# KhutornoyYaroslav/vcm-ts

Measured on AMD Instinct MI355X. Metric: encoded frames/sec at 1920x1080 GOP-32, higher is better.
Workload: dtype f32 (fp16x3 split-MFMA, fp32 accumulate)

## Files before the change

### include/dcvc_hip.h

```cpp
#ifndef DCVC_HIP_H
#define DCVC_HIP_H

#include <stdint.h>

#ifdef __cplusplus
extern "C" {
#endif

#define DCVC_OK 0
#define DCVC_E_ARG (-1)
#define DCVC_E_LAUNCH (-2)
#define DCVC_E_RANGE (-3)

#define DCVC_STATUS_ACT_SATURATED 1

#define DCVC_MAX_SEG 3

#define DCVC_PREC_FP32 0
#define DCVC_PREC_FP16X3 1

typedef struct {
    const float *ptr;
    int32_t C;
    int32_t cs;
} dcvc_seg;

typedef struct {
    dcvc_seg seg[DCVC_MAX_SEG];
    int32_t nseg;
    int32_t N, Hin, Win;
    int32_t in_act;
    float in_slope;
    const float *wpack;
    const float *bpack;
    int32_t ks;
    int32_t stride;
    int32_t Cout;
    int32_t Cout_pad;
    float *out;
    int32_t out_cs;
    int32_t out_act;
    float out_slope;
    int32_t pixel_shuffle;
    const float *res;
    int32_t res_cs;
    const float *res_gate;
    const float *res2;
    int32_t res2_cs;
    int32_t precision;
    int32_t *status;
    float *chan_partial;
    int32_t tile_row0;
    int32_t tile_rows;
    int32_t pair_taps;
} dcvc_conv_args;

int32_t dcvc_conv_tile_rows(int32_t ks, int32_t stride);

int32_t dcvc_conv_chan_partial_parts(int32_t ks, int32_t stride, int32_t Hout, int32_t Wout);
int dcvc_channel_mean_finish(const float *chan_partial, int32_t parts, int32_t row_stride, float *mean, int32_t N,
                             int32_t C, int32_t HW, void *stream);

int64_t dcvc_conv_pack_size(int32_t Cout, int32_t ks, int32_t nseg, const int32_t *seg_C, int32_t *cout_pad);

int dcvc_conv_pack_weights(const float *w, const float *b, int32_t Cout, int32_t ks, int32_t nseg,
                           const int32_t *seg_C, int32_t pixel_shuffle, int32_t precision, float *wpack,
                           float *bpack);

int64_t dcvc_conv_pack_size_paired(int32_t Cout, int32_t Cin, int32_t *cout_pad);
int dcvc_conv_pack_weights_paired(const float *w, const float *b, int32_t Cout, int32_t Cin, float *wpack, float *bpack);

int dcvc_conv2d(const dcvc_conv_args *a, void *stream);
int dcvc_conv_set_lookahead(int32_t mode);

int64_t dcvc_conv_small_pack_bytes(int32_t Cout, int32_t ks, int32_t nseg, const int32_t *seg_C);
int dcvc_conv_small_pack_weights(const float *w, const float *b, int32_t Cout, int32_t ks, int32_t nseg,
                                 const int32_t *seg_C, void *wpack, float *bpack);
int dcvc_conv2d_small(const dcvc_conv_args *a, void *stream);

int64_t dcvc_conv_k32_pack_bytes(int32_t Cout, int32_t ks, int32_t nseg, const int32_t *seg_C, int32_t *cout_pad);
int dcvc_conv_k32_pack_weights(const float *w, const float *b, int32_t Cout, int32_t ks, int32_t nseg,
                               const int32_t *seg_C, int32_t pixel_shuffle, void *wpack, float *bpack);
int dcvc_conv2d_k32(const dcvc_conv_args *a, void *stream);
int dcvc_conv_k32_set_waves(int32_t waves);

int dcvc_warp(const float *src, int32_t src_cs, const float *flow, int32_t flow_cs, float *out, int32_t out_cs,
              int32_t N, int32_t H, int32_t W, int32_t C, void *stream);
int dcvc_up2(const float *src, int32_t src_cs, float *out, int32_t out_cs, float *out2, int32_t out2_cs,
             int32_t N, int32_t H, int32_t W, int32_t C, float scale, void *stream);
int dcvc_down2(const float *src, int32_t src_cs, float *out, int32_t out_cs, int32_t N, int32_t H, int32_t W,
               int32_t C, float scale, int32_t avgpool_order, void *stream);
int dcvc_maxpool2(const float *src, int32_t src_cs, float *out, int32_t out_cs, int32_t N, int32_t H, int32_t W,
                  int32_t C, void *stream);
int dcvc_copy_channels(const float *src, int32_t src_cs, float *out, int32_t out_cs, int64_t npix, int32_t C,
                       void *stream);
int dcvc_nchw_to_nhwc(const float *src, float *out, int32_t out_cs, int32_t N, int32_t C, int32_t H, int32_t W,
                      void *stream);
int dcvc_nhwc_to_nchw(const float *src, int32_t src_cs, float *out, int32_t N, int32_t C, int32_t H, int32_t W,
                      int32_t clamp01, void *stream);

int dcvc_channel_mean(const float *src, int32_t src_cs, float *mean, float *scratch, int32_t N, int32_t HW,
                      int32_t C, void *stream);
int dcvc_se_gate(const float *mean, const float *w1, const float *w2, float *gate, int32_t N, int32_t C,
                 int32_t Cr, void *stream);

int dcvc_scale_channels(const float *src, int32_t src_cs, float *out, int32_t out_cs, const float *q_basic,
                        const float *q_scale, int32_t mode, int32_t N, int32_t HW, int32_t C, void *stream);
int dcvc_scale_channels_map(const float *src, int32_t src_cs, float *out, int32_t out_cs, const float *q_basic,
                            const float *q_scale, int32_t mode, int32_t N, int32_t HW, int32_t C, const float *q_map,
                            int32_t H, int32_t W, void *stream);
int dcvc_round_symbols(const float *z, int32_t z_cs, float *z_hat, int32_t zh_cs, int32_t *sym, int32_t N,
                       int32_t H, int32_t W, int32_t C, void *stream);
int dcvc_symbols_to_nhwc(const int32_t *sym, float *out, int32_t out_cs, int32_t N, int32_t H, int32_t W,
                         int32_t C, void *stream);

typedef struct {
    const float *y;
    int32_t y_cs;
    const float *fusion;
    int32_t fusion_cs;
    const float *spatial;
    int32_t spatial_cs;
    float *params;
    int32_t params_cs;
    float *y_hat;
    float *y_q;
    float *y_res;
    float *scales_hat;
    int32_t *sym;
    int32_t *idx;
    float *out;
    int32_t out_cs;
    const float *q_basic;
    const float *q_scale;
    int32_t N, H, W, C;
    int32_t step;
    const float *idx_edges;
    const float *forced_q;
    const float *q_map;
} dcvc_dual_prior_args;

int dcvc_scale_indexes(const float *scales, int32_t *idx, int64_t n, const float *idx_edges, void *stream);

int dcvc_dual_prior_enc(const dcvc_dual_prior_args *a, void *stream);
int dcvc_dual_prior_dec_index(const dcvc_dual_prior_args *a, void *stream);
int dcvc_dual_prior_dec_apply(const dcvc_dual_prior_args *a, void *stream);

int dcvc_scale_bits(const float *y_q, const float *scales_hat, float *out, float *scratch, int32_t kind, int32_t N,
                    int64_t per_sample, void *stream);
int dcvc_factorized_bits(const float *z_hat, int32_t z_cs, const float *params, float *out, float *scratch, int32_t N,
                         int32_t HW, int32_t C, void *stream);
int dcvc_sq_err(const float *a, int32_t a_cs, const float *b, int32_t b_cs, float *out, float *scratch, int32_t N,
                int32_t HW, int32_t C, void *stream);

int32_t dcvc_cdf_table_cols(void);
int dcvc_build_scale_cdfs(const float *scales, int32_t n_scales, int32_t kind, int32_t *cdf, int32_t *sizes,
// ... 10 lines not shown
```

### vcm_ts_amd/csrc/conv_mfma.hip

```cpp
#include <hip/hip_runtime.h>
#include <stdint.h>
#include <stdlib.h>
#include <string.h>
#include <type_traits>
#include <vector>

#include "dcvc_hip.h"
#include "kernel_common.h"

namespace {

constexpr int LDK = 20;


struct ConvK {
    const float *seg_ptr[DCVC_MAX_SEG];
    int seg_C[DCVC_MAX_SEG];
    int seg_cs[DCVC_MAX_SEG];
    int nseg;
    int Hin, Win, Hout, Wout;
    int in_act;
    float in_slope;
    const float *wpack;
    const float *bpack;
    int Cout, Cout_pad;
    float *out;
    int out_cs;
    int out_act;
    float out_slope;
    int ps;
    const float *res;
    int res_cs;
    const float *res_gate;
    const float *res2;
    int res2_cs;
    int vec_epi;
    int *status;
    float *chan_partial;
    int ntx;
    int ty0, nty;
    int band_rows;
};

int g_lookahead = 2;

inline long dev_env_long(const char *name, long dflt) {
    const char *dev = getenv("DCVC_DEV");
    if (!dev || strcmp(dev, "1") != 0) return dflt;
    const char *v = getenv(name);
    return v ? atol(v) : dflt;
}


template <int KS, int S, int RPW, int NT, bool SPLIT, bool PAIR = false, bool AHEAD = false>
__global__ __launch_bounds__(256, 2) void conv_mfma(const ConvK a) {
    static_assert(!PAIR || (KS == 7 && S == 1 && SPLIT), "tap pairing is built for the 7x7 split-fp16 layers");
    constexpr int BH = 4 * RPW, BW = 32, BN = 32 * NT;
    constexpr int PH = (BH - 1) * S + KS, PW = (BW - 1) * S + KS, PAD = KS / 2;
    constexpr int T = PAIR ? KS * 4 : KS * KS;
    constexpr int TPS = PAIR ? 4 : (KS == 3 && S == 1) ? 9 : KS;
    constexpr int NST = T / TPS;
    constexpr int EPI_LD = BN + 4;
    constexpr int LDS_MAIN = PH * PW * LDK + TPS * 4 * BN * 4, LDS_EPI = 4 * 32 * EPI_LD, LDS_RED = 4 * BN;
    __shared__ __attribute__((aligned(16))) float lds[LDS_MAIN > LDS_EPI + LDS_RED ? LDS_MAIN : LDS_EPI + LDS_RED];
    float *patch = lds;
    float *wl = lds + PH * PW * LDK;

    const int tid = threadIdx.x, lane = tid & 63, wave = tid >> 6;
    const int nbn = a.Cout_pad / BN;
    const int nb = blockIdx.x % nbn, tx = blockIdx.x / nbn;
    if (tx >= a.ntx) return;
    const int ty = blockIdx.y + a.ty0;
    const int x0 = tx * BW, y0 = ty * BH, n0 = nb * BN, img = blockIdx.z;

    f32x16 acc[RPW][NT];
#pragma unroll
    for (int m = 0; m < RPW; ++m)
#pragma unroll
        for (int n = 0; n < NT; ++n)
#pragma unroll
            for (int r = 0; r < 16; ++r) acc[m][n][r] = 0.f;

    const int a_base = ((wave * RPW * S) * PW + (lane & 31) * S) * LDK + (lane >> 5) * 4;
    const int b_base = ((lane >> 5) * BN + (lane & 31)) * 4;

    constexpr int NP = (PH * PW * 4 + 255) / 256, NW = (TPS * 4 * BN + 255) / 256;
    static_assert(!AHEAD || NST >= 3, "AHEAD: two straight-line steps and a loop over the rest of a chunk");
    f32x4 rp[NP], rw[NW];
    struct Cursor {
        int s, c0, cg, st;
    };
    auto advance = [&](Cursor &k) {
        if (++k.st == NST) {
            k.st = 0;
            ++k.cg;
            k.c0 += MFMA_KC;
            if (k.c0 >= a.seg_C[k.s]) {
                ++k.s;
                k.c0 = 0;
            }
        }
    };
    int poff[NP];
    unsigned inpic = 0;
#pragma unroll
    for (int u = 0; u < NP; ++u) {
        const int i = tid + u * 256;
        const int p = i >> 2;
        const int py = p / PW, px = p - py * PW + (PAIR ? (i & 3) >> 1 : 0);
        const int gy = y0 * S - PAD + py, gx = x0 * S - PAD + px;
        const bool ok = i < PH * PW * 4 && gy >= 0 && gy < a.Hin && gx >= 0 && gx < a.Win;
        poff[u] = ok ? gy * a.Win + gx : 0;
        inpic |= (ok ? 1u : 0u) << u;
    }
    auto load_patch = [&](const Cursor &k) {
        const int C = a.seg_C[k.s], cs = a.seg_cs[k.s];
        const float *sp = a.seg_ptr[k.s] + (size_t)img * a.Hin * a.Win * cs;
        const int c = PAIR ? (tid & 1) * 4 : k.c0 + (tid & 3) * 4;
        const int cc = c < C ? c : 0;
#pragma unroll
        for (int u = 0; u < NP; ++u) rp[u] = *(const f32x4 *)(sp + (size_t)poff[u] * cs + cc);
    };
    auto store_patch = [&](const Cursor &k) {
        const int C = a.seg_C[k.s];
#pragma unroll
        for (int u = 0; u < NP; ++u) {
            const int i = tid + u * 256;
            if (i < PH * PW * 4) {
                const int c = PAIR ? (i & 1) * 4 : k.c0 + (i & 3) * 4;
                f32x4 v = ((inpic >> u) & 1u) && c < C ? rp[u] : (f32x4){0.f, 0.f, 0.f, 0.f};
                if (c + 3 >= C) {
                    if (c + 1 >= C) v[1] = 0.f;
                    if (c + 2 >= C) v[2] = 0.f;
                    v[3] = 0.f;
                }
                if (a.in_act) {
                    v[0] = act(v[0], a.in_slope);
                    v[1] = act(v[1], a.in_slope);
                    v[2] = act(v[2], a.in_slope);
                    v[3] = act(v[3], a.in_slope);
                }
                if (!SPLIT) {
                    *(f32x4 *)&patch[(i >> 2) * LDK + (i & 3) * 4] = v;
                } else {
                    f32x4 sv = v * ACT_SCALE;
#pragma unroll
                    for (int e = 0; e < 4; ++e) sv[e] = __builtin_amdgcn_fmed3f(sv[e], -F16_MAX, F16_MAX);
                    const f16x4 hi = __builtin_convertvector(sv, f16x4);
                    const f16x4 lo = __builtin_convertvector(sv - __builtin_convertvector(hi, f32x4), f16x4);
                    _Float16 *rec = (_Float16 *)&patch[(i >> 2) * LDK];
                    *(f16x4 *)&rec[(i & 3) * 4] = hi;
                    *(f16x4 *)&rec[16 + (i & 3) * 4] = lo;
                }
            }
        }
    };
    constexpr int W_OVER = NW * 256 - TPS * 4 * BN;
    static_assert(!AHEAD || TPS * 4 * BN >= W_OVER, "the doubled float4 must lie inside the slab");
    auto w_slot = [&](const int u) {
        const int i = tid + u * 256;
        return AHEAD && W_OVER > 0 && u == NW - 1 && i >= TPS * 4 * BN ? i - W_OVER : i;
    };
    auto load_w = [&](const Cursor &k) {
        const float *wsrc = a.wpack + ((size_t)(k.cg * T + k.st * TPS) * 4) * a.Cout_pad * 4 + (size_t)n0 * 4;
#pragma unroll
        for (int u = 0; u < NW; ++u) {
            const int i = w_slot(u);
            const int row = i / BN, col = i - row * BN;
            if (AHEAD || i < TPS * 4 * BN) rw[u] = *(const f32x4 *)(wsrc + ((size_t)row * a.Cout_pad + col) * 4);
        }
    };
    auto store_w = [&]() {
#pragma unroll
        for (int u = 0; u < NW; ++u) {
            const int i = w_slot(u);
            if (AHEAD || i < TPS * 4 * BN) *(f32x4 *)&wl[i * 4] = rw[u];
        }
    };
    auto mfma_step = [&](const int st) {
        const int a_st = (TPS == T) ? 0 : st * PW * LDK;
#pragma unroll
        for (int tt = 0; tt < TPS; ++tt) {
            const int ky = (TPS == T) ? tt / KS : 0, kx = PAIR ? 2 * tt : (TPS == T) ? tt % KS : tt;
            if (!SPLIT) {
#pragma unroll
                for (int k2 = 0; k2 < 2; ++k2) {
                    f32x4 af[RPW], bf[NT];
#pragma unroll
                    for (int m = 0; m < RPW; ++m)
                        af[m] = *(const f32x4 *)&patch[a_base + a_st + ((m * S + ky) * PW + kx) * LDK + k2 * 8];
#pragma unroll
                    for (int n = 0; n < NT; ++n)
                        bf[n] = *(const f32x4 *)&wl[b_base + ((tt * 4 + k2 * 2) * BN + n * 32) * 4];
#pragma unroll
                    for (int j = 0; j < 4; ++j)
#pragma unroll
                        for (int m = 0; m < RPW; ++m)
#pragma unroll
                            for (int n = 0; n < NT; ++n)
                                acc[m][n] = __builtin_amdgcn_mfma_f32_32x32x2f32(af[m][j], bf[n][j], acc[m][n], 0, 0, 0);
                }
            } else {
                f16x8 ah[RPW], al[RPW], bh[NT], bl[NT];
#pragma unroll
                for (int m = 0; m < RPW; ++m) {
                    const float *rec = &patch[a_base + a_st + ((m * S + ky) * PW + kx) * LDK];
                    ah[m] = *(const f16x8 *)rec;
                    al[m] = *(const f16x8 *)(rec + 8);
                }
#pragma unroll
                for (int n = 0; n < NT; ++n) {
                    bh[n] = *(const f16x8 *)&wl[b_base + ((tt * 4) * BN + n * 32) * 4];
                    bl[n] = *(const f16x8 *)&wl[b_base + ((tt * 4 + 2) * BN + n * 32) * 4];
                }
#pragma unroll
                for (int m = 0; m < RPW; ++m)
#pragma unroll
                    for (int n = 0; n < NT; ++n) {
                        acc[m][n] = __builtin_amdgcn_mfma_f32_32x32x16_f16(ah[m], bh[n], acc[m][n], 0, 0, 0);
                        acc[m][n] = __builtin_amdgcn_mfma_f32_32x32x16_f16(ah[m], bl[n], acc[m][n], 0, 0, 0);
                        acc[m][n] = __builtin_amdgcn_mfma_f32_32x32x16_f16(al[m], bh[n], acc[m][n], 0, 0, 0);
                    }
            }
        }
    };

    Cursor cur = {0, 0, 0, 0};
    if constexpr (AHEAD) {
        auto chunk = [&](auto more, const Cursor &nc) {
            constexpr bool MORE = decltype(more)::value;
            __syncthreads();
            store_patch(cur);
            store_w();
            __syncthreads();
            advance(cur);
            load_w(cur);
            if (MORE) load_patch(nc);
            mfma_step(0);
            auto row_step = [&](const int st) {
                __syncthreads();
                store_w();
                __syncthreads();
                if (st + 1 < NST) {
                    advance(cur);
                    load_w(cur);
                } else if (MORE) {
                    load_w(nc);
                }
                mfma_step(st);
            };
            row_step(1);
            for (int st = 2; st < NST; ++st) row_step(st);
        };
        load_patch(cur);
        load_w(cur);
        for (;;) {
            Cursor nc = cur;
            nc.st = NST - 1;
            advance(nc);
            if (nc.s >= a.nseg) break;
            chunk(std::true_type{}, nc);
            cur = nc;
        }
        chunk(std::false_type{}, cur);
    } else {
        load_patch(cur);
        load_w(cur);
        while (cur.s < a.nseg) {
            __syncthreads();
            if (cur.st == 0) store_patch(cur);
            store_w();
            __syncthreads();
            Cursor nxt = cur;
            advance(nxt);
            if (nxt.s < a.nseg) {
                if (nxt.st == 0) load_patch(nxt);
                load_w(nxt);
            }
            mfma_step(cur.st);
            cur = nxt;
        }
    }

    const int col = lane & 31, hh = lane >> 5;
    const int Cq = a.Cout >> 2;
    const int Cfin = a.ps ? Cq : a.Cout;
    const int Ho = a.ps ? a.Hout * 2 : a.Hout, Wo = a.ps ? a.Wout * 2 : a.Wout;
    const float inv_scale = SPLIT ? 1.f / (ACT_SCALE * WGT_SCALE) : 1.f;
    float vmax = 0.f;
    if (a.vec_epi) {
        constexpr int LPP = BN / 4, PPI = 64 / LPP, NIT = 32 / PPI;
        float *epi = lds + wave * 32 * EPI_LD;
        const int c4 = (lane % LPP) * 4, pl = lane / LPP;
        const int ch = n0 + c4;
        const bool ch_ok = ch < a.Cout;
        int dy = 0, dx = 0, cf = ch;
        if (a.ps) {
            const int sub = ch / Cq;
            cf = ch - sub * Cq;
            dy = sub >> 1;
            dx = sub & 1;
        }
        f32x4 bias = {0.f, 0.f, 0.f, 0.f}, gate = {1.f, 1.f, 1.f, 1.f};
        if (ch_ok) {
            bias = *(const f32x4 *)&a.bpack[ch];
            if (a.res_gate) gate = *(const f32x4 *)&a.res_gate[(size_t)img * Cfin + cf];
        }
        __syncthreads();
        size_t pix[RPW][NIT];
        bool ok[RPW][NIT];
        f32x4 rv[RPW][NIT], rv2[RPW][NIT];
// ... 57 lines not shown
            }
            asm volatile("s_waitcnt lgkmcnt(0)" ::: "memory");
        }
        if (a.status && !(vmax <= ACT_LIMIT)) atomicOr(a.status, DCVC_STATUS_ACT_SATURATED);
        if (a.chan_partial) {
#pragma unroll
            for (int off = LPP; off < 64; off <<= 1)
#pragma unroll
                for (int e = 0; e < 4; ++e) csum[e] += __shfl_xor(csum[e], off);
            float *red = lds + LDS_EPI;
            if (lane < LPP) *(f32x4 *)&red[wave * BN + c4] = csum;
            __syncthreads();
            if (tid < BN && n0 + tid < a.Cout_pad) {
                const float s = ((red[tid] + red[BN + tid]) + red[2 * BN + tid]) + red[3 * BN + tid];
                const size_t part = (size_t)img * (a.nty * a.ntx) + (size_t)ty * a.ntx + tx;
                a.chan_partial[part * a.Cout_pad + n0 + tid] = s;
            }
        }
        return;
    }
#pragma unroll
    for (int m = 0; m < RPW; ++m) {
        const int oy = y0 + wave * RPW + m;
        if (oy >= a.Hout) continue;
#pragma unroll
        for (int n = 0; n < NT; ++n) {
            const int ch = n0 + n * 32 + col;
            if (ch >= a.Cout) continue;
            const float bias = a.bpack[ch];
            int dy = 0, dx = 0, cf = ch;
            if (a.ps) {
                const int sub = ch / Cq;
                cf = ch - sub * Cq;
                dy = sub >> 1;
                dx = sub & 1;
            }
            const float gate = a.res_gate ? a.res_gate[(size_t)img * Cfin + cf] : 1.f;
            float rv[16], rv2[16];
#pragma unroll
            for (int r = 0; r < 16; ++r) {
                const int ox = x0 + (r & 3) + 8 * (r >> 2) + 4 * hh;
                const size_t pix = a.ps ? ((size_t)(img * Ho + 2 * oy + dy) * Wo + 2 * ox + dx)
                                        : ((size_t)(img * Ho + oy) * Wo + ox);
                rv[r] = (a.res && ox < a.Wout) ? a.res[pix * a.res_cs + cf] : 0.f;
                rv2[r] = (a.res2 && ox < a.Wout) ? a.res2[pix * a.res2_cs + cf] : 0.f;
            }
#pragma unroll
            for (int r = 0; r < 16; ++r) {
                const int ox = x0 + (r & 3) + 8 * (r >> 2) + 4 * hh;
                if (ox >= a.Wout) continue;
                float v = acc[m][n][r] * inv_scale + bias;
                if (a.out_act == 1) v = act(v, a.out_slope);
                else if (a.out_act == 2) v = fminf(fmaxf(v, 0.f), 1.f);
                const size_t pix = a.ps ? ((size_t)(img * Ho + 2 * oy + dy) * Wo + 2 * ox + dx)
                                        : ((size_t)(img * Ho + oy) * Wo + ox);
                if (a.out_act == 3) {
                    const float mk = rv2[r] > 0.f ? 1.f : a.out_slope;
                    v = a.res ? __builtin_fmaf(v, mk, rv[r]) : v * mk;
                } else {
                    if (a.res) v = a.res_gate ? __builtin_fmaf(rv[r], gate, v) : v + rv[r];
                    if (a.res2) v = rv2[r] + v;
                }
                if (a.status) vmax = fmaxf(vmax, fabsf(v));
                a.out[pix * a.out_cs + cf] = v;
            }
        }
    }
    if (a.status && !(vmax <= ACT_LIMIT)) atomicOr(a.status, DCVC_STATUS_ACT_SATURATED);
}


template <int KS, int S, int RPW, int NT, bool PAIR = false>
int launch(ConvK &k, int N, hipStream_t st, int precision) {
    constexpr int BH = 4 * RPW, BN = 32 * NT;
    k.ntx = (k.Wout + 31) / 32;
    static const bool xcd_pad = dev_env_long("DCVC_XCD_PAD", 0) != 0;
    unsigned gx = (unsigned)(k.ntx * (k.Cout_pad / BN));
    if (xcd_pad && gx >= 8) gx = (gx + 7) & ~7u;
    k.nty = (k.Hout + BH - 1) / BH;
    if (k.ty0 < 0 || k.ty0 >= k.nty) return DCVC_E_ARG;
    const int rows = k.band_rows > 0 ? (k.band_rows < k.nty - k.ty0 ? k.band_rows : k.nty - k.ty0) : k.nty;
    dim3 grid(gx, (unsigned)rows, (unsigned)N);
    constexpr bool HAS_AHEAD = (KS == 3 && S == 2) || KS == 7;
    if constexpr (HAS_AHEAD) {
        if (g_lookahead == 2) {
            if (PAIR)
                hipLaunchKernelGGL((conv_mfma<KS, S, RPW, NT, true, PAIR, true>), grid, dim3(256), 0, st, k);
            else if (precision == DCVC_PREC_FP16X3)
                hipLaunchKernelGGL((conv_mfma<KS, S, RPW, NT, true, false, true>), grid, dim3(256), 0, st, k);
            else
                hipLaunchKernelGGL((conv_mfma<KS, S, RPW, NT, false, false, !(KS == 7 && RPW == 2 && NT == 2)>), grid, dim3(256), 0, st, k);
            RET_LAUNCH();
        }
    }
    if (PAIR)
        hipLaunchKernelGGL((conv_mfma<KS, S, RPW, NT, true, PAIR>), grid, dim3(256), 0, st, k);
    else if (precision == DCVC_PREC_FP16X3)
        hipLaunchKernelGGL((conv_mfma<KS, S, RPW, NT, true>), grid, dim3(256), 0, st, k);
    else
        hipLaunchKernelGGL((conv_mfma<KS, S, RPW, NT, false>), grid, dim3(256), 0, st, k);
    RET_LAUNCH();
}

}

extern "C" int64_t dcvc_conv_pack_size(int32_t Cout, int32_t ks, int32_t nseg, const int32_t *seg_C, int32_t *cout_pad) {
    if (Cout <= 0 || nseg <= 0 || nseg > DCVC_MAX_SEG || (ks != 1 && ks != 3 && ks != 7)) return DCVC_E_ARG;
    int chunks = 0;
    for (int s = 0; s < nseg; ++s) chunks += (seg_C[s] + MFMA_KC - 1) / MFMA_KC;
    const int cp = round_up(Cout, 32);
    if (cout_pad) *cout_pad = cp;
    return (int64_t)chunks * ks * ks * 4 * cp * 4;
}

extern "C" int dcvc_conv_pack_weights(const float *w, const float *b, int32_t Cout, int32_t ks, int32_t nseg,
                                      const int32_t *seg_C, int32_t pixel_shuffle, int32_t precision, float *wpack,
                                      float *bpack) {
    if (precision != DCVC_PREC_FP32 && precision != DCVC_PREC_FP16X3) return DCVC_E_ARG;
    int32_t cp = 0;
    const int64_t total = dcvc_conv_pack_size(Cout, ks, nseg, seg_C, &cp);
    if (total < 0 || (pixel_shuffle && (Cout & 3))) return DCVC_E_ARG;
    const int T = ks * ks;
    int Cin = 0;
    for (int s = 0; s < nseg; ++s) Cin += seg_C[s];
    memset(wpack, 0, (size_t)total * sizeof(float));
    memset(bpack, 0, (size_t)cp * sizeof(float));
    const int Cq = Cout / 4;
    _Float16 *base = (_Float16 *)wpack;
    int cg = 0, cin0 = 0;
    for (int s = 0; s < nseg; ++s) {
        for (int c0 = 0; c0 < seg_C[s]; c0 += MFMA_KC, ++cg) {
            for (int t = 0; t < T; ++t)
                for (int cc = 0; cc < MFMA_KC && c0 + cc < seg_C[s]; ++cc)
                    for (int n = 0; n < Cout; ++n) {
                        const int np = pixel_shuffle ? ps_packed_channel(n, Cq) : n;
                        const float v = w[((size_t)n * Cin + cin0 + c0 + cc) * T + t];
                        if (precision == DCVC_PREC_FP32) {
                            wpack[mfma_wpack_f32(cg, T, t, cc, cp, np)] = v;
                        } else {
                            float sv = v * WGT_SCALE;
                            sv = sv > F16_MAX ? F16_MAX : (sv < -F16_MAX ? -F16_MAX : sv);
                            const SplitF16 p = split_f16(sv);
                            base[mfma_wpack_f16(cg, T, t, cc, cp, np, 0)] = p.hi;
                            base[mfma_wpack_f16(cg, T, t, cc, cp, np, 1)] = p.lo;
                        }
                    }
        }
        cin0 += seg_C[s];
    }
    for (int n = 0; n < Cout; ++n) bpack[pixel_shuffle ? ps_packed_channel(n, Cq) : n] = b ? b[n] : 0.f;
    return DCVC_OK;
}

extern "C" int64_t dcvc_conv_pack_size_paired(int32_t Cout, int32_t Cin, int32_t *cout_pad) {
    if (Cout <= 0 || Cin <= 0 || Cin > 8) return DCVC_E_ARG;
    const int cp = round_up(Cout, 32);
    if (cout_pad) *cout_pad = cp;
    return (int64_t)7 * 4 * 4 * cp * 4;
}

extern "C" int dcvc_conv_pack_weights_paired(const float *w, const float *b, int32_t Cout, int32_t Cin, float *wpack, float *bpack) {
    int32_t cp = 0;
    const int64_t total = dcvc_conv_pack_size_paired(Cout, Cin, &cp);
    if (total < 0 || !w || !wpack || !bpack) return DCVC_E_ARG;
    memset(wpack, 0, (size_t)total * sizeof(float));
    memset(bpack, 0, (size_t)cp * sizeof(float));
    _Float16 *base = (_Float16 *)wpack;
    bool clamped = false;
    for (int ky = 0; ky < 7; ++ky)
        for (int kx = 0; kx < 7; ++kx) {
            const int step = ky * 4 + (kx >> 1), h = kx & 1;
            for (int c = 0; c < Cin; ++c)
                for (int n = 0; n < Cout; ++n) {
                    float sv = w[((size_t)n * Cin + c) * 49 + ky * 7 + kx] * WGT_SCALE;
                    if (!(fabsf(sv) <= F16_MAX)) { clamped = true; sv = sv > 0.f ? F16_MAX : -F16_MAX; }
                    const SplitF16 p = split_f16(sv);
                    base[mfma_wpack_f16(0, 28, step, 8 * h + c, cp, n, 0)] = p.hi;
                    base[mfma_wpack_f16(0, 28, step, 8 * h + c, cp, n, 1)] = p.lo;
                }
        }
    for (int n = 0; n < Cout; ++n) bpack[n] = b ? b[n] : 0.f;
    return clamped ? DCVC_E_RANGE : DCVC_OK;
}

static int tile_rows(int ks, int stride) { return stride == 2 ? 4 : 8; }

extern "C" int32_t dcvc_conv_tile_rows(int32_t ks, int32_t stride) { return tile_rows(ks, stride); }

extern "C" int32_t dcvc_conv_chan_partial_parts(int32_t ks, int32_t stride, int32_t Hout, int32_t Wout) {
    if (Hout <= 0 || Wout <= 0 || (stride != 1 && stride != 2)) return DCVC_E_ARG;
    const int bh = tile_rows(ks, stride);
    return ((Wout + 31) / 32) * ((Hout + bh - 1) / bh);
}

extern "C" int dcvc_conv_set_lookahead(int32_t mode) {
    if (mode != 1 && mode != 2) return DCVC_E_ARG;
    g_lookahead = mode;
    return DCVC_OK;
}

extern "C" int dcvc_conv2d(const dcvc_conv_args *a, void *stream) {
    if (!conv_args_ok(a)) return DCVC_E_ARG;
    if (a->stride != 1 && a->stride != 2) return DCVC_E_ARG;
    if (a->precision != DCVC_PREC_FP32 && a->precision != DCVC_PREC_FP16X3) return DCVC_E_ARG;
    if (a->Cout_pad % 32 || a->Cout > a->Cout_pad || (a->pixel_shuffle && (a->Cout & 3))) return DCVC_E_ARG;
    if (a->out_act < 0 || a->out_act > 3) return DCVC_E_ARG;
    if (a->out_act == 3 && (!a->res2 || a->res_gate || a->chan_partial || a->pixel_shuffle)) return DCVC_E_ARG;
    ConvK k;
    memset(&k, 0, sizeof(k));
    copy_conv_args_full(k, a);
    k.Hin = a->Hin;
    k.Win = a->Win;
    const int pad = a->ks / 2;
    k.Hout = (a->Hin + 2 * pad - a->ks) / a->stride + 1;
    k.Wout = (a->Win + 2 * pad - a->ks) / a->stride + 1;
    k.vec_epi = vec_epilogue_ok(a);
    if (a->chan_partial && (!k.vec_epi || a->pixel_shuffle)) return DCVC_E_ARG;
    hipStream_t st = (hipStream_t)stream;
    const bool wide = (a->Cout_pad % 64) == 0;
    const int key = a->ks * 10 + a->stride;
    if (a->stride == 1 && !a->pair_taps && !a->chan_partial && a->tile_rows <= 0) {
        const long wgs8 = (long)((k.Wout + 31) / 32) * ((k.Hout + 7) / 8) * (a->Cout_pad / (wide ? 64 : 32)) * a->N;
        static const long rows4_below = dev_env_long("DCVC_ROWS4_WGS", 384);
        if (wgs8 < rows4_below) {
            if (a->ks == 3) return wide ? launch<3, 1, 1, 2>(k, a->N, st, a->precision) : launch<3, 1, 1, 1>(k, a->N, st, a->precision);
            if (a->ks == 7) return wide ? launch<7, 1, 1, 2>(k, a->N, st, a->precision) : launch<7, 1, 1, 1>(k, a->N, st, a->precision);
            if (a->ks == 1) return wide ? launch<1, 1, 1, 2>(k, a->N, st, a->precision) : launch<1, 1, 1, 1>(k, a->N, st, a->precision);
        }
    }
    switch (key) {
        case 11: return wide ? launch<1, 1, 2, 2>(k, a->N, st, a->precision) : launch<1, 1, 2, 1>(k, a->N, st, a->precision);
        case 12: return wide ? launch<1, 2, 1, 2>(k, a->N, st, a->precision) : launch<1, 2, 1, 1>(k, a->N, st, a->precision);
        case 31:
            return wide ? launch<3, 1, 2, 2>(k, a->N, st, a->precision) : launch<3, 1, 2, 1>(k, a->N, st, a->precision);
        case 32: return wide ? launch<3, 2, 1, 2>(k, a->N, st, a->precision) : launch<3, 2, 1, 1>(k, a->N, st, a->precision);
        case 71:
            if (a->pair_taps) {
                if (a->nseg != 1 || a->seg[0].C > 8 || a->precision != DCVC_PREC_FP16X3 || a->pixel_shuffle) return DCVC_E_ARG;
                return wide ? launch<7, 1, 2, 2, true>(k, a->N, st, a->precision) : launch<7, 1, 2, 1, true>(k, a->N, st, a->precision);
            }
            return wide ? launch<7, 1, 2, 2>(k, a->N, st, a->precision) : launch<7, 1, 2, 1>(k, a->N, st, a->precision);
        default: return DCVC_E_ARG;
    }
}
```

### vcm_ts_amd/lib.py

```python
from __future__ import annotations

import ctypes as C
import functools
import os

HERE = os.path.dirname(os.path.abspath(__file__))
CSRC = os.path.join(HERE, "csrc")


class LibraryMissing(RuntimeError):
    pass


class KernelError(RuntimeError):
    pass


def _load(name):
    path = os.environ.get("DCVC_HIP_LIB") if name == "libdcvc_hip.so" and os.environ.get("DCVC_HIP_LIB") else \
        os.path.join(CSRC, name)
    if not os.path.exists(path):
        raise LibraryMissing(f"{path} not built; run `make -C {CSRC}` (no CPU fallback exists)")
    return C.CDLL(path)

# ... 38 lines not shown
class DualPriorArgs(C.Structure):
    _fields_ = [
        ("y", C.c_void_p), ("y_cs", C.c_int32), ("fusion", C.c_void_p), ("fusion_cs", C.c_int32),
        ("spatial", C.c_void_p), ("spatial_cs", C.c_int32), ("params", C.c_void_p), ("params_cs", C.c_int32),
        ("y_hat", C.c_void_p), ("y_q", C.c_void_p), ("y_res", C.c_void_p), ("scales_hat", C.c_void_p),
        ("sym", C.c_void_p), ("idx", C.c_void_p), ("out", C.c_void_p), ("out_cs", C.c_int32),
        ("q_basic", C.c_void_p), ("q_scale", C.c_void_p), ("N", C.c_int32), ("H", C.c_int32), ("W", C.c_int32),
        ("C", C.c_int32), ("step", C.c_int32), ("idx_edges", C.c_void_p), ("forced_q", C.c_void_p),
        ("q_map", C.c_void_p),
    ]


class ConvBwdArgs(C.Structure):
    _fields_ = [
        ("dout", C.c_void_p), ("dout_cs", C.c_int32), ("out", C.c_void_p), ("out_cs", C.c_int32),
        ("res", C.c_void_p), ("res_cs", C.c_int32), ("gate", C.c_void_p), ("res2", C.c_void_p), ("res2_cs", C.c_int32),
        ("dres", C.c_void_p), ("dres_cs", C.c_int32), ("dres2", C.c_void_p), ("dres2_cs", C.c_int32),
        ("dpre", C.c_void_p), ("dpre_cs", C.c_int32), ("zs", C.c_int32), ("Hd", C.c_int32), ("Wd", C.c_int32),
        ("N", C.c_int32), ("Ho", C.c_int32), ("Wo", C.c_int32), ("Cout", C.c_int32), ("pixel_shuffle", C.c_int32),
        ("act", C.c_int32), ("slope", C.c_float),
    ]


class WgradArgs(C.Structure):
    _fields_ = [
        ("x", C.c_void_p), ("x_cs", C.c_int32), ("C", C.c_int32), ("in_act", C.c_int32), ("in_slope", C.c_float),
        ("dpre", C.c_void_p), ("dpre_cs", C.c_int32), ("zs", C.c_int32), ("Hd", C.c_int32), ("Wd", C.c_int32),
        ("N", C.c_int32), ("Hin", C.c_int32), ("Win", C.c_int32), ("Ho", C.c_int32), ("Wo", C.c_int32),
        ("Cout", C.c_int32), ("ks", C.c_int32), ("stride", C.c_int32), ("dw", C.c_void_p), ("Cin_total", C.c_int32),
        ("cin_offset", C.c_int32), ("scratch", C.c_void_p), ("scratch_floats", C.c_int64), ("overwrite", C.c_int32),
        ("db", C.c_void_p), ("precision", C.c_int32),
    ]


class PackJob(C.Structure):
    _fields_ = [
        ("w", C.c_void_p), ("b", C.c_void_p), ("Cout", C.c_int32), ("Cin_total", C.c_int32), ("ks", C.c_int32),
        ("nseg", C.c_int32), ("seg_C", C.c_int32 * 3), ("cin_offset", C.c_int32), ("pixel_shuffle", C.c_int32),
        ("precision", C.c_int32), ("transposed", C.c_int32), ("wpack", C.c_void_p), ("bpack", C.c_void_p),
    ]


class DualPriorBwdArgs(C.Structure):
    _fields_ = [
        ("y", C.c_void_p), ("y_cs", C.c_int32), ("fusion", C.c_void_p), ("fusion_cs", C.c_int32),
        ("y_hat", C.c_void_p), ("dout", C.c_void_p), ("dout_cs", C.c_int32), ("dy_res", C.c_void_p),
        ("dscales_hat", C.c_void_p), ("dparams", C.c_void_p), ("dparams_cs", C.c_int32),
        ("dspatial", C.c_void_p), ("dspatial_cs", C.c_int32), ("dy", C.c_void_p), ("dy_cs", C.c_int32),
        ("dfusion", C.c_void_p), ("dfusion_cs", C.c_int32), ("dq_plane", C.c_void_p),
        ("q_basic", C.c_void_p), ("q_scale", C.c_void_p), ("N", C.c_int32), ("H", C.c_int32), ("W", C.c_int32),
        ("C", C.c_int32), ("step", C.c_int32),
    ]


class ColorCoeffs(C.Structure):
    _fields_ = [(n, C.c_float) for n in ("y_off", "c_off", "y_scale", "c_scale", "crr", "cgb", "cgr", "cbb", "kr", "kg", "kb",
                                         "icb", "icr", "y_range", "c_range")] + \
               [(n, C.c_int32) for n in ("max_code", "bit_depth", "siting", "matrix", "range")]


class RoiBox(C.Structure):
    _fields_ = [(n, C.c_int32) for n in ("x1", "y1", "x2", "y2", "cls")]


class RoiClassRec(C.Structure):
    _fields_ = [("border", C.c_int32), ("shrink", C.c_int32), ("feather", C.c_float * 64)]


PRECISIONS = {"fp32": 0, "fp16x3": 1}

i32, i64, f32, vp = C.c_int32, C.c_int64, C.c_float, C.c_void_p

HEADERS = {
    "dcvc_hip.h": {
        "dcvc_conv_tile_rows": (i32, i32, i32),
        "dcvc_conv_chan_partial_parts": (i32, i32, i32, i32, i32),
        "dcvc_channel_mean_finish": [vp, i32, i32, vp, i32, i32, i32, vp],
        "dcvc_conv_pack_size": (i64, i32, i32, i32, vp, C.POINTER(i32)),
        "dcvc_conv_pack_weights": [vp, vp, i32, i32, i32, vp, i32, i32, vp, vp],
        "dcvc_conv_pack_size_paired": (i64, i32, i32, C.POINTER(i32)),
        "dcvc_conv_pack_weights_paired": [vp, vp, i32, i32, vp, vp],
        "dcvc_conv2d": [C.POINTER(ConvArgs), vp],
        "dcvc_conv_set_lookahead": [i32],
        "dcvc_conv_small_pack_bytes": (i64, i32, i32, i32, vp),
        "dcvc_conv_small_pack_weights": [vp, vp, i32, i32, i32, vp, vp, vp],
        "dcvc_conv2d_small": [C.POINTER(ConvArgs), vp],
        "dcvc_conv_k32_pack_bytes": (i64, i32, i32, i32, vp, C.POINTER(i32)),
        "dcvc_conv_k32_pack_weights": [vp, vp, i32, i32, i32, vp, i32, vp, vp],
        "dcvc_conv2d_k32": [C.POINTER(ConvArgs), vp],
        "dcvc_conv_k32_set_waves": [i32],
        "dcvc_warp": [vp, i32, vp, i32, vp, i32, i32, i32, i32, i32, vp],
        "dcvc_up2": [vp, i32, vp, i32, vp, i32, i32, i32, i32, i32, f32, vp],
        "dcvc_down2": [vp, i32, vp, i32, i32, i32, i32, i32, f32, i32, vp],
        "dcvc_maxpool2": [vp, i32, vp, i32, i32, i32, i32, i32, vp],
        "dcvc_copy_channels": [vp, i32, vp, i32, i64, i32, vp],
        "dcvc_nchw_to_nhwc": [vp, vp, i32, i32, i32, i32, i32, vp],
        "dcvc_nhwc_to_nchw": [vp, i32, vp, i32, i32, i32, i32, i32, vp],
        "dcvc_channel_mean": [vp, i32, vp, vp, i32, i32, i32, vp],
        "dcvc_se_gate": [vp, vp, vp, vp, i32, i32, i32, vp],
        "dcvc_scale_channels": [vp, i32, vp, i32, vp, vp, i32, i32, i32, i32, vp],
        "dcvc_scale_channels_map": [vp, i32, vp, i32, vp, vp, i32, i32, i32, i32, vp, i32, i32, vp],
        "dcvc_round_symbols": [vp, i32, vp, i32, vp, i32, i32, i32, i32, vp],
        "dcvc_symbols_to_nhwc": [vp, vp, i32, i32, i32, i32, i32, vp],
        "dcvc_scale_indexes": [vp, vp, i64, vp, vp],
        "dcvc_dual_prior_enc": [C.POINTER(DualPriorArgs), vp],
        "dcvc_dual_prior_dec_index": [C.POINTER(DualPriorArgs), vp],
        "dcvc_dual_prior_dec_apply": [C.POINTER(DualPriorArgs), vp],
        "dcvc_scale_bits": [vp, vp, vp, vp, i32, i32, i64, vp],
        "dcvc_factorized_bits": [vp, i32, vp, vp, vp, i32, i32, i32, vp],
        "dcvc_sq_err": [vp, i32, vp, i32, vp, vp, i32, i32, i32, vp],
        "dcvc_cdf_table_cols": (i32,),
        "dcvc_build_scale_cdfs": [vp, i32, i32, vp, vp, vp, vp],
        "dcvc_build_factorized_cdfs": [vp, i32, vp, vp, vp, vp],
        "dcvc_hip_version": (C.c_char_p,),
    },
    "dcvc_hip_grad.h": {
        "dcvc_conv_pack_weights_dev": [vp, vp, i32, i32, i32, i32, vp, i32, i32, i32, i32, vp, vp, vp],
        "dcvc_pack_plan_create": [C.POINTER(PackJob), i32, C.POINTER(C.c_void_p)],
        "dcvc_pack_plan_run": [vp, vp],
        "dcvc_pack_plan_destroy": (None, vp),
        "dcvc_conv_bwd_prologue": [C.POINTER(ConvBwdArgs), vp],
        "dcvc_conv_wgrad_scratch_min": (i64, i32, i32, i32),
        "dcvc_conv_wgrad": [C.POINTER(WgradArgs), vp],
        "dcvc_channel_dot": [vp, i32, vp, i32, vp, vp, i32, i32, i32, i32, i32, vp],
        "dcvc_mask_accumulate": [vp, i32, vp, i32, f32, vp, i32, i64, i32, vp],
        "dcvc_add_planes": [vp, i32, vp, i32, vp, i32, i64, i32, vp],
        "dcvc_warp_bwd": [vp, i32, vp, i32, vp, i32, vp, i32, vp, i32, i32, i32, i32, i32, vp, vp],
        "dcvc_up2_bwd": [vp, i32, vp, i32, i32, i32, i32, i32, f32, vp],
        "dcvc_down2_bwd": [vp, i32, vp, i32, i32, i32, i32, i32, f32, vp],
        "dcvc_maxpool2_bwd": [vp, i32, vp, i32, vp, i32, i32, i32, i32, i32, vp],
        "dcvc_se_bwd": [vp, vp, vp, vp, vp, vp, vp, vp, i32, i32, i32, vp],
        "dcvc_add_channel_vec": [vp, i32, vp, f32, i32, i32, i32, vp],
        "dcvc_scale_channels_bwd": [vp, i32, vp, i32, vp, vp, i32, i32, i32, i32, vp],
        "dcvc_q_finish": [vp, vp, vp, vp, vp, vp, i32, i32, vp],
        "dcvc_dual_prior_bwd": [C.POINTER(DualPriorBwdArgs), vp],
        "dcvc_scale_bits_bwd": [vp, vp, vp, vp, vp, i32, i32, i64, vp],
        "dcvc_factorized_bits_bwd": [vp, i32, vp, vp, vp, i32, vp, i32, i32, i32, vp],
        "dcvc_sq_err_bwd": [vp, i32, vp, i32, vp, vp, i32, i32, i32, i32, vp],
    },
    "dcvc_hip_rans.h": {
        "dcvc_drans_default_lanes": (i32, i64),
        "dcvc_drans_scratch_words": (i64, i64, i32),
        "dcvc_drans_build_lut": [vp, i32, i32, vp, vp],
        "dcvc_drans_encode": [vp, vp, i32, i32, i64, vp, i32, i32, vp, vp, i32, vp, i64, vp, i64, vp, vp, vp, vp],
        "dcvc_drans_decode": [vp, i64, vp, vp, vp, i32, i32, i64, vp, i32, i32, vp, vp, vp, i32, vp, vp, vp],
    },
    "dcvc_hip_metrics.h": {
        "dcvc_ms_ssim": [vp, vp, i32, i32, i32, i32, i32, i64, i32, i64, f32, i32, vp, vp, vp, vp, vp],
        "dcvc_ms_ssim_grad": [vp, vp, i32, i32, i32, i32, i32, i64, i32, i64, f32, i32, vp, vp, vp, vp],
        "dcvc_ms_ssim_workspace_bytes": (i64, i32, i32, i32, i32, i32),
    },
    "dcvc_hip_color.h": {
        "dcvc_color_coeffs": [i32, i32, i32, i32, vp],
        "dcvc_yuv420_to_rgb": [vp, vp, vp, i32, i32, i32, i32, vp, vp, i32, i32, i32, i64, i32, vp],
        "dcvc_rgb_to_yuv420": [vp, i32, i32, i32, i64, vp, vp, vp, vp, i32, i32, vp, vp, vp, i32, i32, vp, vp],
    },
    "dcvc_hip_roi.h": {
        "dcvc_roi_residual": [vp, i32, i64, vp, i32, i64, i32, i32, vp, vp, i32, vp, i64, i64, i32, i32, i32, i32, vp],
        "dcvc_roi_fuse": [vp, i32, i64, vp, i64, i64, i32, i32, i32, i32, i32, i32, vp, vp, i32, vp, i32, vp, i32, i64, vp],
        "dcvc_roi_sse": [vp, i32, i64, vp, i32, i64, i32, i32, vp, vp, i32, vp, i32, vp, vp],
        "dcvc_roi_qmap": [i32, i32, vp, vp, i32, i32, vp, i32, vp, vp],
    },
    "dcvc_hip_roil.h": {
        "dcvc_roil_cells": [i32, i32, vp, i32, vp, vp, i32],
        "dcvc_roil_check": [vp, i64, vp, i32],
        "dcvc_roil_encode": [vp, i32, i64, vp, i32, i64, i32, i32, vp, vp, i32, i32, vp, i32, vp, vp, i64, vp, vp],
# ... 74 lines not shown
```

Measured before the change: 42.91.

## Stage two filter rows per pipeline step in lookahead MFMA conv

Adds an RPS template parameter so the lookahead conv kernel stages weights for two filter rows per step instead of one. This halves the number of barrier-separated steps per channel chunk for 3x3 stride-2 and 7x7 layers. The intent is to cut __syncthreads and store/load round trips and give the MFMA stream longer runs between barriers. The cost is a larger LDS weight slab, which the code checks still lets two workgroups share a CU. It is on by default through a new step_rows global set to 2, with a setter to switch back to one row per step.

After: 43.02, median of 6. No clear change (+0.3%).

```diff
diff --git a/include/dcvc_hip.h b/include/dcvc_hip.h
--- a/include/dcvc_hip.h
+++ b/include/dcvc_hip.h
@@ -72,6 +72,7 @@
 
 int dcvc_conv2d(const dcvc_conv_args *a, void *stream);
 int dcvc_conv_set_lookahead(int32_t mode);
+int dcvc_conv_set_step_rows(int32_t rows);
 
 int64_t dcvc_conv_small_pack_bytes(int32_t Cout, int32_t ks, int32_t nseg, const int32_t *seg_C);
 int dcvc_conv_small_pack_weights(const float *w, const float *b, int32_t Cout, int32_t ks, int32_t nseg,
diff --git a/vcm_ts_amd/csrc/conv_mfma.hip b/vcm_ts_amd/csrc/conv_mfma.hip
--- a/vcm_ts_amd/csrc/conv_mfma.hip
+++ b/vcm_ts_amd/csrc/conv_mfma.hip
@@ -42,7 +42,24 @@
     int band_rows;
 };
 
-int g_lookahead = 2;
+}
+
+extern "C" {
+int dcvc_conv_lookahead_mode = 2;
+int dcvc_conv_step_rows = 2;
+}
+
+namespace {
+
+constexpr int step_filter_rows(int ks, int rps, int st) { return ks - st * rps < rps ? ks - st * rps : rps; }
+
+template <int FROM, int TO, class F>
+__device__ __forceinline__ void static_for(F &&f) {
+    if constexpr (FROM < TO) {
+        f(std::integral_constant<int, FROM>{});
+        static_for<FROM + 1, TO>(f);
+    }
+}
 
 inline long dev_env_long(const char *name, long dflt) {
     const char *dev = getenv("DCVC_DEV");
@@ -52,17 +69,20 @@
 }
 
 
-template <int KS, int S, int RPW, int NT, bool SPLIT, bool PAIR = false, bool AHEAD = false>
+template <int KS, int S, int RPW, int NT, bool SPLIT, bool PAIR = false, bool AHEAD = false, int RPS = 1>
 __global__ __launch_bounds__(256, 2) void conv_mfma(const ConvK a) {
     static_assert(!PAIR || (KS == 7 && S == 1 && SPLIT), "tap pairing is built for the 7x7 split-fp16 layers");
     constexpr int BH = 4 * RPW, BW = 32, BN = 32 * NT;
     constexpr int PH = (BH - 1) * S + KS, PW = (BW - 1) * S + KS, PAD = KS / 2;
     constexpr int T = PAIR ? KS * 4 : KS * KS;
-    constexpr int TPS = PAIR ? 4 : (KS == 3 && S == 1) ? 9 : KS;
-    constexpr int NST = T / TPS;
+    constexpr int ROWT = PAIR ? 4 : KS;
+    constexpr int TPS = (KS == 3 && S == 1) ? 9 : RPS * ROWT;
+    constexpr int NST = (KS == 3 && S == 1) ? 1 : (KS + RPS - 1) / RPS;
+    static_assert(RPS == 1 || (AHEAD && RPS == 2 && NST >= 2), "two filter rows per step are built on the AHEAD schedule");
     constexpr int EPI_LD = BN + 4;
     constexpr int LDS_MAIN = PH * PW * LDK + TPS * 4 * BN * 4, LDS_EPI = 4 * 32 * EPI_LD, LDS_RED = 4 * BN;
     __shared__ __attribute__((aligned(16))) float lds[LDS_MAIN > LDS_EPI + LDS_RED ? LDS_MAIN : LDS_EPI + LDS_RED];
+    static_assert(RPS == 1 || sizeof(lds) <= 160 * 1024 / 2, "two filter rows per step only where two workgroups stay on a CU");
     float *patch = lds;
     float *wl = lds + PH * PW * LDK;
 
@@ -85,7 +105,7 @@
     const int b_base = ((lane >> 5) * BN + (lane & 31)) * 4;
 
     constexpr int NP = (PH * PW * 4 + 255) / 256, NW = (TPS * 4 * BN + 255) / 256;
-    static_assert(!AHEAD || NST >= 3, "AHEAD: two straight-line steps and a loop over the rest of a chunk");
+    static_assert(!AHEAD || RPS > 1 || NST >= 3, "AHEAD: two straight-line steps and a loop over the rest of a chunk");
     f32x4 rp[NP], rw[NW];
     struct Cursor {
         int s, c0, cg, st;
@@ -177,56 +197,122 @@
             if (AHEAD || i < TPS * 4 * BN) *(f32x4 *)&wl[i * 4] = rw[u];
         }
     };
+    auto mfma_tap = [&](const int a_off, const int wt) __attribute__((always_inline)) {
+        if (!SPLIT) {
+#pragma unroll
+            for (int k2 = 0; k2 < 2; ++k2) {
+                f32x4 af[RPW], bf[NT];
+#pragma unroll
+                for (int m = 0; m < RPW; ++m)
+                    af[m] = *(const f32x4 *)&patch[a_base + a_off + m * S * PW * LDK + k2 * 8];
+#pragma unroll
+                for (int n = 0; n < NT; ++n)
+                    bf[n] = *(const f32x4 *)&wl[b_base + ((wt * 4 + k2 * 2) * BN + n * 32) * 4];
+#pragma unroll
+                for (int j = 0; j < 4; ++j)
+#pragma unroll
+                    for (int m = 0; m < RPW; ++m)
+#pragma unroll
+                        for (int n = 0; n < NT; ++n)
+                            acc[m][n] = __builtin_amdgcn_mfma_f32_32x32x2f32(af[m][j], bf[n][j], acc[m][n], 0, 0, 0);
+            }
+        } else {
+            f16x8 ah[RPW], al[RPW], bh[NT], bl[NT];
+#pragma unroll
+            for (int m = 0; m < RPW; ++m) {
+                const float *rec = &patch[a_base + a_off + m * S * PW * LDK];
+                ah[m] = *(const f16x8 *)rec;
+                al[m] = *(const f16x8 *)(rec + 8);
+            }
+#pragma unroll
+            for (int n = 0; n < NT; ++n) {
+                bh[n] = *(const f16x8 *)&wl[b_base + ((wt * 4) * BN + n * 32) * 4];
+                bl[n] = *(const f16x8 *)&wl[b_base + ((wt * 4 + 2) * BN + n * 32) * 4];
+            }
+#pragma unroll
+            for (int m = 0; m < RPW; ++m)
+#pragma unroll
+                for (int n = 0; n < NT; ++n) {
+                    acc[m][n] = __builtin_amdgcn_mfma_f32_32x32x16_f16(ah[m], bh[n], acc[m][n], 0, 0, 0);
+                    acc[m][n] = __builtin_amdgcn_mfma_f32_32x32x16_f16(ah[m], bl[n], acc[m][n], 0, 0, 0);
+                    acc[m][n] = __builtin_amdgcn_mfma_f32_32x32x16_f16(al[m], bh[n], acc[m][n], 0, 0, 0);
+                }
+        }
+    };
     auto mfma_step = [&](const int st) {
         const int a_st = (TPS == T) ? 0 : st * PW * LDK;
 #pragma unroll
         for (int tt = 0; tt < TPS; ++tt) {
             const int ky = (TPS == T) ? tt / KS : 0, kx = PAIR ? 2 * tt : (TPS == T) ? tt % KS : tt;
-            if (!SPLIT) {
-#pragma unroll
-                for (int k2 = 0; k2 < 2; ++k2) {
-                    f32x4 af[RPW], bf[NT];
-#pragma unroll
-                    for (int m = 0; m < RPW; ++m)
-                        af[m] = *(const f32x4 *)&patch[a_base + a_st + ((m * S + ky) * PW + kx) * LDK + k2 * 8];
-#pragma unroll
-                    for (int n = 0; n < NT; ++n)
-                        bf[n] = *(const f32x4 *)&wl[b_base + ((tt * 4 + k2 * 2) * BN + n * 32) * 4];
-#pragma unroll
-                    for (int j = 0; j < 4; ++j)
-#pragma unroll
-                        for (int m = 0; m < RPW; ++m)
-#pragma unroll
-                            for (int n = 0; n < NT; ++n)
-                                acc[m][n] = __builtin_amdgcn_mfma_f32_32x32x2f32(af[m][j], bf[n][j], acc[m][n], 0, 0, 0);
-                }
-            } else {
-                f16x8 ah[RPW], al[RPW], bh[NT], bl[NT];
-#pragma unroll
-                for (int m = 0; m < RPW; ++m) {
-                    const float *rec = &patch[a_base + a_st + ((m * S + ky) * PW + kx) * LDK];
-                    ah[m] = *(const f16x8 *)rec;
-                    al[m] = *(const f16x8 *)(rec + 8);
-                }
-#pragma unroll
-                for (int n = 0; n < NT; ++n) {
-                    bh[n] = *(const f16x8 *)&wl[b_base + ((tt * 4) * BN + n * 32) * 4];
-                    bl[n] = *(const f16x8 *)&wl[b_base + ((tt * 4 + 2) * BN + n * 32) * 4];
-                }
-#pragma unroll
-                for (int m = 0; m < RPW; ++m)
-#pragma unroll
-                    for (int n = 0; n < NT; ++n) {
-                        acc[m][n] = __builtin_amdgcn_mfma_f32_32x32x16_f16(ah[m], bh[n], acc[m][n], 0, 0, 0);
-                        acc[m][n] = __builtin_amdgcn_mfma_f32_32x32x16_f16(ah[m], bl[n], acc[m][n], 0, 0, 0);
-                        acc[m][n] = __builtin_amdgcn_mfma_f32_32x32x16_f16(al[m], bh[n], acc[m][n], 0, 0, 0);
-                    }
-            }
+            mfma_tap(a_st + (ky * PW + kx) * LDK, tt);
         }
     };
 
     Cursor cur = {0, 0, 0, 0};
-    if constexpr (AHEAD) {
+    if constexpr (AHEAD && RPS > 1) {
+        auto load_w_n = [&](const int cg, auto stc) __attribute__((always_inline)) {
+            constexpr int ST = decltype(stc)::value, CNT = step_filter_rows(KS, RPS, ST) * ROWT * 4 * BN;
+            constexpr int NWS = (CNT + 255) / 256, OVER = NWS * 256 - CNT;
+            static_assert(CNT >= OVER && NWS <= NW, "the doubled float4 must lie inside the slab");
+            const float *wsrc = a.wpack + ((size_t)(cg * T + ST * TPS) * 4) * a.Cout_pad * 4 + (size_t)n0 * 4;
+#pragma unroll
+            for (int u = 0; u < NWS; ++u) {
+                const int i0 = tid + u * 256, i = OVER > 0 && u == NWS - 1 && i0 >= CNT ? i0 - OVER : i0;
+                const int row = i / BN, col = i - row * BN;
+                rw[u] = *(const f32x4 *)(wsrc + ((size_t)row * a.Cout_pad + col) * 4);
+            }
+        };
+        auto store_w_n = [&](auto stc) __attribute__((always_inline)) {
+            constexpr int ST = decltype(stc)::value, CNT = step_filter_rows(KS, RPS, ST) * ROWT * 4 * BN;
+            constexpr int NWS = (CNT + 255) / 256, OVER = NWS * 256 - CNT;
+#pragma unroll
+            for (int u = 0; u < NWS; ++u) {
+                const int i0 = tid + u * 256, i = OVER > 0 && u == NWS - 1 && i0 >= CNT ? i0 - OVER : i0;
+                *(f32x4 *)&wl[i * 4] = rw[u];
+            }
+        };
+        auto mfma_rows = [&](auto stc) __attribute__((always_inline)) {
+            constexpr int ST = decltype(stc)::value, NR = step_filter_rows(KS, RPS, ST);
+#pragma unroll
+            for (int r = 0; r < NR; ++r)
+#pragma unroll
+                for (int tt = 0; tt < ROWT; ++tt)
+                    mfma_tap(((ST * RPS + r) * PW + (PAIR ? 2 * tt : tt)) * LDK, r * ROWT + tt);
+        };
+        constexpr std::integral_constant<int, 0> st0{};
+        auto chunk = [&](auto more, const Cursor &nc) __attribute__((always_inline)) {
+            constexpr bool MORE = decltype(more)::value;
+            __syncthreads();
+            store_patch(cur);
+            store_w_n(st0);
+            __syncthreads();
+            load_w_n(cur.cg, std::integral_constant<int, 1>{});
+            if (MORE) load_patch(nc);
+            mfma_rows(st0);
+            static_for<1, NST>([&](auto stc) __attribute__((always_inline)) {
+                constexpr int ST = decltype(stc)::value;
+                __syncthreads();
+                store_w_n(stc);
+                __syncthreads();
+                if constexpr (ST + 1 < NST)
+                    load_w_n(cur.cg, std::integral_constant<int, ST + 1>{});
+                else if (MORE)
+                    load_w_n(nc.cg, st0);
+                mfma_rows(stc);
+            });
+        };
+        load_patch(cur);
+        load_w_n(0, st0);
+        for (;;) {
+            Cursor nc = cur;
+            nc.st = NST - 1;
+            advance(nc);
+            if (nc.s >= a.nseg) break;
+            chunk(std::true_type{}, nc);
+            cur = nc;
+        }
+        chunk(std::false_type{}, cur);
+    } else if constexpr (AHEAD) {
         auto chunk = [&](auto more, const Cursor &nc) {
             constexpr bool MORE = decltype(more)::value;
             __syncthreads();
@@ -450,8 +536,18 @@
     const int rows = k.band_rows > 0 ? (k.band_rows < k.nty - k.ty0 ? k.band_rows : k.nty - k.ty0) : k.nty;
     dim3 grid(gx, (unsigned)rows, (unsigned)N);
     constexpr bool HAS_AHEAD = (KS == 3 && S == 2) || KS == 7;
+    constexpr bool TWO_ROWS = !PAIR && ((KS == 3 && S == 2 && NT == 2) || (KS == 7 && RPW == 2 && NT == 1));
+    if constexpr (TWO_ROWS) {
+        if (dcvc_conv_lookahead_mode == 2 && dcvc_conv_step_rows == 2) {
+            if (precision == DCVC_PREC_FP16X3)
+                hipLaunchKernelGGL((conv_mfma<KS, S, RPW, NT, true, false, true, 2>), grid, dim3(256), 0, st, k);
+            else
+                hipLaunchKernelGGL((conv_mfma<KS, S, RPW, NT, false, false, true, 2>), grid, dim3(256), 0, st, k);
+            RET_LAUNCH();
+        }
+    }
     if constexpr (HAS_AHEAD) {
-        if (g_lookahead == 2) {
+        if (dcvc_conv_lookahead_mode == 2) {
             if (PAIR)
                 hipLaunchKernelGGL((conv_mfma<KS, S, RPW, NT, true, PAIR, true>), grid, dim3(256), 0, st, k);
             else if (precision == DCVC_PREC_FP16X3)
@@ -563,7 +659,13 @@
 
 extern "C" int dcvc_conv_set_lookahead(int32_t mode) {
     if (mode != 1 && mode != 2) return DCVC_E_ARG;
-    g_lookahead = mode;
+    dcvc_conv_lookahead_mode = mode;
+    return DCVC_OK;
+}
+
+extern "C" int dcvc_conv_set_step_rows(int32_t rows) {
+    if (rows != 1 && rows != 2) return DCVC_E_ARG;
+    dcvc_conv_step_rows = rows;
     return DCVC_OK;
 }
 
diff --git a/vcm_ts_amd/lib.py b/vcm_ts_amd/lib.py
--- a/vcm_ts_amd/lib.py
+++ b/vcm_ts_amd/lib.py
@@ -144,6 +144,7 @@
         "dcvc_conv_pack_weights_paired": [vp, vp, i32, i32, vp, vp],
         "dcvc_conv2d": [C.POINTER(ConvArgs), vp],
         "dcvc_conv_set_lookahead": [i32],
+        "dcvc_conv_set_step_rows": [i32],
         "dcvc_conv_small_pack_bytes": (i64, i32, i32, i32, vp),
         "dcvc_conv_small_pack_weights": [vp, vp, i32, i32, i32, vp, vp, vp],
         "dcvc_conv2d_small": [C.POINTER(ConvArgs), vp],
```
